# dmiruke/find_motion

Measured on NVIDIA B200. Metric: 1080p frames/sec (whole box), higher is better.
Workload: dtype u8+f64

## Files before the change

### find_motion_b200/csrc/fm_host.cu

```cuda
#include <ctype.h>
#include <math.h>
#include <stdarg.h>
#include <stdio.h>
#include <stdlib.h>
#include <string.h>

#include <algorithm>
#include <map>
#include <mutex>
#include <utility>
#include <vector>

#include <sched.h>
#include <unistd.h>

#include "fm_common.cuh"

std::atomic<unsigned long long> g_launches{0};
static thread_local char g_err[512] = "";

int fm_ensure_smem(const void *func, size_t bytes, int device) {
    static std::mutex mu;
    static std::map<std::pair<const void *, int>, size_t> done;
    std::lock_guard<std::mutex> lk(mu);
// ... 274 lines not shown
        if ((rc = upload(&c->coef, taps))) return fail(rc);
        if (c->umma && (rc = fm_umma_init(c, taps.data()))) return fail(rc);
        if (!c->fused && !c->umma && (rc = fm_wide_init(c, taps.data()))) return fail(rc);
    }

    const size_t F = (size_t)c->S * c->Tmax;
    const size_t flatw = (size_t)c->ntiles * FM_TILE_WORDS;
#define ALLOC(ptr, bytes)                                                                 \
    do {                                                                                  \
        cudaError_t e_ = cudaMalloc((void **)&(ptr), (bytes));                            \
        if (e_ != cudaSuccess) {                                                          \
            fm_set_error("cudaMalloc(%zu bytes) for %s failed: %s", (size_t)(bytes), #ptr, \
                         cudaGetErrorString(e_));                                         \
            return fail(FM_ENOMEM);                                                       \
        }                                                                                 \
    } while (0)
    const bool keep = (cfg->flags & FM_FLAG_KEEP_PLANES) != 0;
    const bool need_gray = keep || !c->fused;
    const bool need_blur = keep || !c->fused;
    ALLOC(c->gray, need_gray ? F * c->N : 16);
    ALLOC(c->hor, (c->fused || c->umma) ? 16 : 2 * fm_wide_plane_bytes(c));
    ALLOC(c->blur, need_blur ? F * c->N + 64 : 64);
    const size_t bg_doubles = std::max((size_t)c->S * c->ntiles * FM_TILE_PX,
                                       c->fused ? fm_fused_bg_doubles(c)
                                                : (c->umma ? fm_umma_bg_doubles(c) : (c->wide_fused ? fm_wide_bg_doubles(c) : (size_t)0)));
    ALLOC(c->bg, bg_doubles * sizeof(double));
    ALLOC(c->maskbits, (size_t)c->S * c->h * c->wpr * 4);
    ALLOC(c->maskflat, (size_t)c->S * flatw * 4);
    ALLOC(c->tflat, (F * flatw + FM_TILE_WORDS) * 4);
    ALLOC(c->dil, F * c->h * c->wpr * 4);
    ALLOC(c->fill, F * c->h * c->wpr * 4);
    ALLOC(c->rawrange, F * 6 * sizeof(int));
    c->any = c->rawrange + 2 * F;
    ALLOC(c->ncomp, (F * 2 + 4) * sizeof(int));
    c->ncounted = c->ncomp + F;
    ALLOC(c->heavy, F * sizeof(int));
    ALLOC(c->comps, F * c->maxc * sizeof(fm_component));
    ALLOC(c->stats, F * sizeof(fm_frame_stats));
    ALLOC(c->state, (size_t)c->S * sizeof(StreamState));
    ALLOC(c->errflag, sizeof(int));
    ALLOC(c->nvalid, (size_t)c->S * sizeof(int));
    c->nvalid_host = (int *)malloc((size_t)c->S * sizeof(int));
    if (!c->nvalid_host) { fm_set_error("out of host memory"); return fail(FM_ENOMEM); }
    for (int s = 0; s < c->S; s++) c->nvalid_host[s] = c->Tmax;
    FM_TRY(cudaMemcpy(c->nvalid, c->nvalid_host, (size_t)c->S * sizeof(int), cudaMemcpyHostToDevice));
    FM_TRY(cudaMemset(c->maskbits, 0, (size_t)c->S * c->h * c->wpr * 4));
    FM_TRY(cudaMemset(c->maskflat, 0, (size_t)c->S * flatw * 4));
    FM_TRY(cudaMemset(c->tflat, 0, (F * flatw + FM_TILE_WORDS) * 4));
    FM_TRY(cudaMemset(c->bg, 0, bg_doubles * sizeof(double)));
    FM_TRY(cudaMemset(c->state, 0, (size_t)c->S * sizeof(StreamState)));
    FM_TRY(cudaMemset(c->errflag, 0, sizeof(int)));
    FM_TRY(cudaMemset(c->heavy, 0, F * sizeof(int)));
    int cap = c->w / 4 + 3;
    size_t per_frame = (size_t)c->h * cap * 28 + (size_t)c->h * 4 + 4;
    size_t budget = (size_t)8 << 30;
    int nb = (int)std::min<size_t>(F, std::max<size_t>(1, budget / per_frame));
    if ((rc = fm_ccl_alloc(&c->ccl, nb, c->h, cap))) return fail(rc);
    if ((rc = fm_ccl_configure(c))) return fail(rc);
    if ((cfg->flags & FM_FLAG_DEVICE_CLIPS) && (rc = fm_clips_alloc(c))) return fail(rc);
    FM_TRY(cudaStreamCreateWithFlags(&c->own_stream, cudaStreamNonBlocking));
    FM_TRY(cudaStreamCreateWithFlags(&c->copy_stream, cudaStreamNonBlocking));
    for (int i = 0; i < 2; i++) {
        FM_TRY(cudaEventCreateWithFlags(&c->ev_copied[i], cudaEventDisableTiming));
        FM_TRY(cudaEventCreateWithFlags(&c->ev_done[i], cudaEventDisableTiming));
    }
#undef FM_TRY
#undef ALLOC
// ... 30 lines not shown
    if (err) {
        FM_CUDA(cudaMemset(c->errflag, 0, sizeof(int)));
        fm_set_error("contour stage: run capacity exceeded (results of the affected frames are not valid)");
        return FM_ERANGE;
    }
    return FM_OK;
}

extern "C" int fm_ctx_set_masks(fm_ctx *c, int stream, int n_polys, const int32_t *poly_offsets,
                                const int32_t *xy) {
    if (!c || n_polys < 0 || (n_polys > 0 && (!poly_offsets || !xy))) { fm_set_error("bad mask arguments"); return FM_EINVAL; }
    if (stream >= c->S) { fm_set_error("stream %d out of range", stream); return FM_EINVAL; }
    FM_CUDA(cudaSetDevice(c->cfg.device));
    FM_CUDA(cudaDeviceSynchronize());
    int npts = n_polys ? poly_offsets[n_polys] : 0;
    std::vector<int> pts((size_t)npts * 2);
    const double scale = c->info.scale;
    for (int i = 0; i < npts * 2; i++) pts[i] = (int)((double)xy[i] * scale);
    int s0 = stream < 0 ? 0 : stream, s1 = stream < 0 ? c->S : stream + 1;
    for (int s = s0; s < s1; s++) {
        int rc = fm_launch_masks(c, s, n_polys, poly_offsets, pts.data(), npts, 0);
        if (rc) return rc;
    }
    FM_CUDA(cudaDeviceSynchronize());
    return FM_OK;
}

static int timing_drain(fm_ctx *c) {
    for (int i = 0; i < c->ev_pending; i++) {
        cudaEvent_t *ev = c->evs + 4 * i;
        FM_CUDA(cudaEventSynchronize(ev[3]));
        for (int g = 0; g < 3; g++) {
            float ms = 0;
            FM_CUDA(cudaEventElapsedTime(&ms, ev[g], ev[g + 1]));
            c->t_ms[g] += ms;
        }
        c->t_calls++;
    }
    c->ev_pending = 0;
    return FM_OK;
}

static int process(fm_ctx *c, const uint8_t *frames, size_t stream_stride, size_t frame_stride, int n_frames,
                   const int32_t *n_valid, void *cuda_stream, fm_frame_stats *stats_dev, uint8_t *out, size_t out_stride) {
    if (!c || !frames) { fm_set_error("null argument"); return FM_EINVAL; }
    if (n_frames < 1 || n_frames > c->Tmax) {
        fm_set_error("n_frames %d outside [1, max_frames=%d]", n_frames, c->Tmax);
        return FM_EINVAL;
    }
    FM_CUDA(cudaSetDevice(c->cfg.device));
    cudaStream_t st = (cudaStream_t)cuda_stream;
    int rc;
    {
        bool changed = false;
        for (int s = 0; s < c->S; s++) {
            int v = n_valid ? n_valid[s] : n_frames;
            if (v < 0 || v > n_frames) { fm_set_error("n_valid[%d] = %d outside [0, n_frames=%d]", s, v, n_frames); return FM_EINVAL; }
            if (v != c->nvalid_host[s]) { c->nvalid_host[s] = v; changed = true; }
        }
        if (changed) FM_CUDA(cudaMemcpyAsync(c->nvalid, c->nvalid_host, (size_t)c->S * sizeof(int), cudaMemcpyHostToDevice, st));
    }
    {
        const size_t Fmax = (size_t)c->S * c->Tmax;
        FM_CUDA(cudaMemsetAsync(c->rawrange, 0xFF, Fmax * 6 * sizeof(int), st));
        FM_CUDA(cudaMemsetAsync(c->ncomp, 0, (Fmax * 2 + 4) * sizeof(int), st));
    }
    cudaEvent_t *ev = nullptr;
    if (c->timing) {
        if (c->ev_pending == FM_TIMING_RING && (rc = timing_drain(c))) return rc;
        ev = c->evs + 4 * c->ev_pending++;
        FM_CUDA(cudaEventRecord(ev[0], st));
    }
    if (c->fused) {
        if ((rc = fm_launch_fused(c, frames, stream_stride, frame_stride, n_frames, st))) return rc;
        if (ev) { FM_CUDA(cudaEventRecord(ev[1], st)); FM_CUDA(cudaEventRecord(ev[2], st)); }
    } else {
        if ((rc = fm_launch_frontend(c, frames, stream_stride, frame_stride, n_frames, st))) return rc;
        if (ev) FM_CUDA(cudaEventRecord(ev[1], st));
        if (!c->wide_fused && !c->umma && (rc = fm_launch_temporal(c, n_frames, st))) return rc;
        if (ev) FM_CUDA(cudaEventRecord(ev[2], st));
    }
    if ((rc = fm_launch_morph_ccl(c, n_frames, st, stats_dev))) return rc;
    if (ev) FM_CUDA(cudaEventRecord(ev[3], st));
    if ((c->cfg.flags & FM_FLAG_DEVICE_CLIPS) &&
        (rc = fm_launch_clips(c, frames, stream_stride, frame_stride, n_frames, out, out_stride, st)))
        return rc;
    c->last_T = n_frames;
    c->planes_valid = true;
    return FM_OK;
}

extern "C" int fm_process_ragged(fm_ctx *c, const uint8_t *frames, size_t stream_stride, size_t frame_stride,
                                 int n_frames, const int32_t *n_valid, void *cuda_stream, fm_frame_stats *stats_dev) {
    return process(c, frames, stream_stride, frame_stride, n_frames, n_valid, cuda_stream, stats_dev, nullptr, 0);
}

extern "C" int fm_process_clip(fm_ctx *c, const uint8_t *frames, size_t stream_stride, size_t frame_stride,
                               int n_frames, const int32_t *n_valid, void *cuda_stream, fm_frame_stats *stats_dev,
                               uint8_t *out_dev, size_t out_stream_stride, int out_capacity) {
    if (!c || !frames || !out_dev) { fm_set_error("null argument"); return FM_EINVAL; }
    if (!(c->cfg.flags & FM_FLAG_DEVICE_CLIPS)) {
        fm_set_error("fm_process_clip needs a context created with FM_FLAG_DEVICE_CLIPS");
        return FM_EINVAL;
    }
    if ((long long)out_capacity < (long long)c->info.cache_frames + n_frames) {
        fm_set_error("out_capacity %d < cache_frames %d + n_frames %d (the most frames one call can write)", out_capacity,
                     c->info.cache_frames, n_frames);
        return FM_EINVAL;
// ... 341 lines not shown
```

### find_motion_b200/csrc/k_morph_ccl.cu

```cuda
#include "fm_common.cuh"

#define WARPS_PER_BLOCK 8

__device__ __forceinline__ uint32_t ld_word(const uint32_t *row, int j, int wpr) {
    return ((unsigned)j < (unsigned)wpr) ? __ldg(row + j) : 0u;
}

__device__ __forceinline__ uint32_t flat_row_word(const uint32_t *flat, int y, int j, int w, int h, int wpr) {
    if ((unsigned)y >= (unsigned)h || (unsigned)j >= (unsigned)wpr) return 0u;
    long long b0 = (long long)y * w + 32 * j;
    int wi = (int)(b0 >> 5), sh = (int)(b0 & 31);
    uint32_t lo = __ldg(flat + wi);
    uint32_t v = lo;
    if (sh) {
        uint32_t hi = __ldg(flat + wi + 1);
        v = __funnelshift_r(lo, hi, sh);
    }
    int rem = w - 32 * j;
    if (rem < 32) v &= (1u << rem) - 1u;
    return v;
}

template <bool ALIGNED>
__device__ __forceinline__ uint32_t dilate_vor(const uint32_t *__restrict__ flat, int y, int j, int w, int h, int wpr) {
    uint32_t v = 0;
    if (j >= wpr) return 0u;
#pragma unroll
    for (int dy = -2; dy <= 2; dy++) {
        const int yy = y + dy;
        if (ALIGNED) {
            if ((unsigned)yy < (unsigned)h) v |= __ldcg(flat + (size_t)yy * wpr + j);
        } else {
            v |= flat_row_word(flat, yy, j, w, h, wpr);
        }
    }
    return v;
}

template <bool ALIGNED>
__device__ __forceinline__ uint32_t dilate_row(const uint32_t *__restrict__ flat, uint32_t *__restrict__ out, int y, int w,
                                               int h, int wpr, int lane, int &jmin, int &jmax) {
    uint32_t anyw = 0, vprev = 0, vc = dilate_vor<ALIGNED>(flat, y, lane, w, h, wpr);
    for (int j0 = 0; j0 < wpr; j0 += 32) {
        const int j = j0 + lane;
        const uint32_t vnext = dilate_vor<ALIGNED>(flat, y, j + 32, w, h, wpr);
        uint32_t vm = __shfl_up_sync(0xffffffffu, vc, 1), vp = __shfl_down_sync(0xffffffffu, vc, 1);
        const uint32_t pl = __shfl_sync(0xffffffffu, vprev, 31), nf = __shfl_sync(0xffffffffu, vnext, 0);
        if (lane == 0) vm = pl;
        if (lane == 31) vp = nf;
        if (j < wpr) {
            uint32_t d = vc | (vc << 1) | (vc << 2) | (vc >> 1) | (vc >> 2) | (vm >> 31) | (vm >> 30) | (vp << 31) | (vp << 30);
            const int rem = w - 32 * j;
            if (rem < 32) d &= (1u << rem) - 1u;
            out[j] = d;
            anyw |= d;
            if (d) { jmax = max(jmax, j); jmin = min(jmin, j); }
        }
        vprev = vc;
        vc = vnext;
    }
    return anyw;
}

template <bool ALIGNED, int NCH>
__device__ __noinline__ void dilate_rows(const uint32_t *flat, uint32_t *dplane, int ya, int yb, int w, int h, int wpr, int lane,
                                            int &jmin, int &jmax, int &ymn, int &ymx) {
    auto raw = [&](int y, int c) -> uint32_t {
        const int j = lane + 32 * c;
        if ((unsigned)y >= (unsigned)h || j >= wpr) return 0u;
        return ALIGNED ? __ldcg(flat + (size_t)y * wpr + j) : flat_row_word(flat, y, j, w, h, wpr);
    };
    uint32_t win[NCH][4];
#pragma unroll
    for (int c = 0; c < NCH; c++)
#pragma unroll
        for (int i = 0; i < 4; i++) win[c][i] = raw(ya - 2 + i, c);
    for (int y0 = ya; y0 < yb; y0 += 4) {
        uint32_t nxt[NCH][4];
#pragma unroll
        for (int c = 0; c < NCH; c++)
#pragma unroll
            for (int i = 0; i < 4; i++) nxt[c][i] = raw(y0 + 2 + i, c);
#pragma unroll
        for (int i = 0; i < 4; i++) {
            const int y = y0 + i;
            if (y >= yb) break;
            uint32_t v[NCH];
#pragma unroll
            for (int c = 0; c < NCH; c++) {
                v[c] = win[c][0] | win[c][1] | win[c][2] | win[c][3] | nxt[c][i];
                win[c][0] = win[c][1]; win[c][1] = win[c][2]; win[c][2] = win[c][3]; win[c][3] = nxt[c][i];
            }
            uint32_t anyw = 0;
#pragma unroll
            for (int c = 0; c < NCH; c++) {
                uint32_t vm = __shfl_up_sync(0xffffffffu, v[c], 1), vp = __shfl_down_sync(0xffffffffu, v[c], 1);
                const uint32_t pl = c > 0 ? __shfl_sync(0xffffffffu, v[c > 0 ? c - 1 : 0], 31) : 0u;
                const uint32_t nf = c + 1 < NCH ? __shfl_sync(0xffffffffu, v[c + 1 < NCH ? c + 1 : c], 0) : 0u;
                if (lane == 0) vm = pl;
                if (lane == 31) vp = nf;
                const int j = lane + 32 * c;
                if (j < wpr) {
                    uint32_t d = v[c] | (v[c] << 1) | (v[c] << 2) | (v[c] >> 1) | (v[c] >> 2) | (vm >> 31) | (vm >> 30) | (vp << 31) | (vp << 30);
                    const int rem = w - 32 * j;
                    if (rem < 32) d &= (1u << rem) - 1u;
                    dplane[(size_t)y * wpr + j] = d;
                    anyw |= d;
                    if (d) { jmax = max(jmax, j); jmin = min(jmin, j); }
                }
            }
            if (__any_sync(0xffffffffu, anyw != 0)) { ymx = max(ymx, y); ymn = min(ymn, y); }
        }
    }
}

template <bool ALIGNED>
__global__ void __launch_bounds__(32 * WARPS_PER_BLOCK) k_dilate(const uint32_t *__restrict__ tflat,
                                                                 uint32_t *__restrict__ dil, int *__restrict__ rowrange,
                                                                 const int *__restrict__ rawrange, int F, int w, int h,
                                                                 int wpr, int flatwords, int T, int t0, int Th) {
    int warp = blockIdx.x * WARPS_PER_BLOCK + (threadIdx.x >> 5);
    int lane = threadIdx.x & 31;
    if (warp >= F * h) return;
    int lf = warp / h, y = warp - lf * h;
    int f = (lf / Th) * T + t0 + lf % Th;
    if (rawrange) {
        int rmax = rawrange[2 * f], rmin = h - 1 - rawrange[2 * f + 1];
        if (rmax < 0 || y < rmin - 3 || y > rmax + 3) return;
    }
    const uint32_t *flat = tflat + (size_t)f * flatwords;
    uint32_t *out = dil + ((size_t)f * h + y) * wpr;
    int jmax = -1, jmin = wpr;
    const uint32_t anyw = dilate_row<ALIGNED>(flat, out, y, w, h, wpr, lane, jmin, jmax);
    if (__any_sync(0xffffffffu, anyw != 0)) {
        jmax = __reduce_max_sync(0xffffffffu, jmax);
        jmin = __reduce_min_sync(0xffffffffu, jmin);
        if (lane == 0) {
            atomicMax(rowrange + 4 * f, y);
            atomicMax(rowrange + 4 * f + 1, h - 1 - y);
            atomicMax(rowrange + 4 * f + 2, jmax);
            atomicMax(rowrange + 4 * f + 3, wpr - 1 - jmin);
        }
    }
}

struct CclArgs {
    const uint32_t *plane;
    uint32_t *fill;
    const int *rowrange;
    const uint32_t *raw;
    const int *rawrange;
    int *rangeout;
    uint32_t *planeout;
    int flatwords, aligned;
    int cache_words;
    int f0, nf;
    int T, t0, Th;
    int w, h, wpr, cap;
    size_t slots;
    uint16_t *xs, *xe;
    int *rowcnt, *parent, *area2, *bbox;
    int *errflag;
    int *ncomp, *ncounted;
    fm_component *comps;
    int maxc, min_area, max_area;
};

template <bool INVERT>
__device__ __forceinline__ uint32_t plane_word(const uint32_t *row, int j, int w, int wpr) {
    if ((unsigned)j >= (unsigned)wpr) return 0u;
    uint32_t v = __ldcg(row + j);
    if (INVERT) {
        v = ~v;
        int rem = w - 32 * j;
        if (rem < 32) v &= (1u << rem) - 1u;
    }
    return v;
}

template <bool INVERT>
__device__ __forceinline__ void runs_row(const CclArgs &a, const uint32_t *plane, int lf, int f, int y, int lane) {
    const uint32_t *row = plane + ((size_t)f * a.h + y) * a.wpr;
    size_t base = (size_t)lf * a.slots + (size_t)y * a.cap;
    int *parent = a.parent + (size_t)lf * (a.slots + 1);
    int nstart = 0, nend = 0;
    for (int j0 = 0; j0 < a.wpr; j0 += 32) {
        int j = j0 + lane;
        uint32_t B = plane_word<INVERT>(row, j, a.w, a.wpr);
        uint32_t Bp = plane_word<INVERT>(row, j - 1, a.w, a.wpr);
        uint32_t Bn = plane_word<INVERT>(row, j + 1, a.w, a.wpr);
        uint32_t S = B & ~((B << 1) | (Bp >> 31));
        uint32_t E = B & ~((B >> 1) | (Bn << 31));
        if (!__any_sync(0xffffffffu, (S | E) != 0)) continue;
        int cs = __popc(S), ce = __popc(E);
        int ps = cs, pe = ce;
#pragma unroll
        for (int o = 1; o < 32; o <<= 1) {
            int vs = __shfl_up_sync(0xffffffffu, ps, o);
            int ve = __shfl_up_sync(0xffffffffu, pe, o);
// ... 154 lines not shown
        if (slot < a.maxc) {
            fm_component c;
            c.area_x2 = area2;
            int x0 = __ldcg(bb), y0 = __ldcg(bb + 1), x1 = __ldcg(bb + 2), y1 = __ldcg(bb + 3);
            c.x = x0; c.y = y0; c.w = x1 - x0 + 1; c.h = y1 - y0 + 1;
            a.comps[(size_t)f * a.maxc + slot] = c;
        }
    }
}

#define CCL_THREADS 1024
__device__ __forceinline__ void ccl_frame_global(const CclArgs &a, int lf, int f, int ylo, int yhi) {
    const int lane = threadIdx.x & 31, warp = threadIdx.x >> 5, nw = CCL_THREADS / 32;
    if (threadIdx.x == 0) a.parent[(size_t)lf * (a.slots + 1)] = 0;
    for (int y = ylo + warp; y <= yhi; y += nw) runs_row<true>(a, a.plane, lf, f, y, lane);
    __syncthreads();
    for (int y = ylo + warp; y <= yhi; y += nw) union_row<false, true>(a, lf, y, ylo, lane);
    __syncthreads();
    for (int y = ylo + warp; y <= yhi; y += nw) fill_row(a, lf, f, y, lane);
    __syncthreads();
    for (int y = ylo + warp; y <= yhi; y += nw) runs_row<false>(a, a.fill, lf, f, y, lane);
    __syncthreads();
    for (int y = ylo + warp; y <= yhi; y += nw) union_row<true, false>(a, lf, y, ylo, lane);
    __syncthreads();
    for (int y = ylo + warp; y <= yhi; y += nw) stats_row(a, lf, f, y, lane);
    __syncthreads();
    for (int y = ylo + warp; y <= yhi; y += nw) collect_row(a, lf, f, y, lane);
}

struct DecideArgs {
    StreamState *state;
    fm_frame_stats *stats, *stats_out;
    const int *nvalid;
    int *done;
    int S, T, total, cache_frames, min_movement_frames;
};

__device__ __forceinline__ void decide_stream(const DecideArgs &d, const int *ncomp, const int *ncounted, int s) {
    StreamState st = d.state[s];
    const int T = d.T;
    const int Ts = min(T, d.nvalid[s]);
    for (int t = Ts; t < T; t++) {
        fm_frame_stats z = {0, 0, 0, 0, 0, 0, 0, 0};
        d.stats[s * T + t] = z;
        if (d.stats_out) d.stats_out[s * T + t] = z;
    }
    if (Ts <= 0) return;
    for (int tc = 0; tc < Ts; tc += 16) {
        int nco[16], ncd[16];
#pragma unroll
        for (int i = 0; i < 16; i++) {
            const bool in = tc + i < Ts;
            nco[i] = in ? __ldcg(ncomp + s * T + tc + i) : 0;
            ncd[i] = in ? __ldcg(ncounted + s * T + tc + i) : 0;
        }
#pragma unroll
        for (int i = 0; i < 16; i++) {
            if (tc + i >= Ts) break;
            const int f = s * T + tc + i;
            fm_frame_stats r;
            r.n_contours = nco[i];
            r.n_counted = ncd[i];
            if (st.decay > 0) st.decay -= 1;
            bool movement = r.n_counted > 0;
            st.counter = movement ? st.counter + r.n_counted : 0;
            r.wrote = 0;
            r.n_flush = 0;
            if (st.counter >= d.min_movement_frames || st.decay > 0) {
                if (movement) {
                    st.decay = d.cache_frames;
                    r.n_flush = st.cache_len;
                    st.cache_len = 0;
                }
                r.wrote = 1;
            } else {
                st.cache_len = min(st.cache_len + 1, d.cache_frames);
            }
            r.movement = movement ? 1 : 0;
            r.movement_counter = st.counter;
            r.movement_decay = st.decay;
            r.cache_len = st.cache_len;
            d.stats[f] = r;
            if (d.stats_out) d.stats_out[f] = r;
        }
    }
    st.has_bg = 1;
    d.state[s] = st;
}

__global__ void k_decide(DecideArgs d, const int *__restrict__ ncomp, const int *__restrict__ ncounted) {
    int s = blockIdx.x * blockDim.x + threadIdx.x;
    if (s < d.S) decide_stream(d, ncomp, ncounted, s);
}

__global__ void __launch_bounds__(CCL_THREADS, 1) k_ccl_frame(CclArgs a, const int *__restrict__ heavy) {
    const int lf = blockIdx.x, lg = a.f0 + lf, f = (lg / a.Th) * a.T + a.t0 + lg % a.Th;
    if (heavy && !heavy[f]) return;
    int ylo = 0, yhi = a.h - 1;
    bool work = true;
    if (a.rowrange) {
        int ymax = a.rowrange[4 * f], ymin = a.h - 1 - a.rowrange[4 * f + 1];
        if (ymax < 0) work = false;
        ylo = max(ymin - 1, 0);
        yhi = min(ymax + 1, a.h - 1);
    }
    if (work) ccl_frame_global(a, lf, f, ylo, yhi);
}

#define CCL2_THREADS 1024
#define CCL2_WARPS (CCL2_THREADS / 32)
#define CCL2_CAP 4096

struct RunTable {
    int2 *row;
    int *parent;
    uint16_t *xs, *xe;
    uint16_t *rowof;
};

__device__ __forceinline__ int suf_find(int *parent, int x) {
    int p = parent[x];
    while (p != x) {
        int gp = parent[p];
        if (gp != p) atomicMin(parent + x, gp);
        x = p;
        p = gp;
    }
    return x;
}

// ... 99 lines not shown
    while (lo < hi) {
        const int mid = (lo + hi) >> 1;
        if ((int)t.xe[prv.x + mid] < xs - d) lo = mid + 1; else hi = mid;
    }
    for (int q = lo; q < prv.y && (int)t.xs[prv.x + q] <= xe + d; q++) {
        if (!linked) {
            if (FIRST) t.parent[id] = id0 + prv.x + q;
            linked = true;
        } else if (!FIRST) {
            suf_union(t.parent, id, id0 + prv.x + q);
            did = true;
        }
    }
    return did;
}

__device__ __forceinline__ void flatten_forest(int *parent, int n) {
    __syncthreads();
    while (true) {
        bool ch = false;
        for (int i = threadIdx.x; i < n; i += CCL2_THREADS) {
            const int p = parent[i];
            int q = parent[p];
            if (q != p) {
                q = parent[parent[q]];
                parent[i] = q;
                ch = true;
            }
        }
        if (!__syncthreads_or(ch)) break;
    }
}

__device__ __forceinline__ bool ccl_frame_lanes(const CclArgs &a, unsigned char *csm, int f, int lf,
                                                int ylo, int yhi, int jlo, int wprw) {
    const int ww = min(a.w - 32 * jlo, 32 * wprw);
    const int nrows = yhi - ylo + 1;
    RunTable bg, fg;
    bg.row = reinterpret_cast<int2 *>(csm);
    fg.row = bg.row + a.h;
    bg.parent = reinterpret_cast<int *>(fg.row + a.h);
    fg.parent = bg.parent + CCL2_CAP + 2;
    bg.xs = reinterpret_cast<uint16_t *>(fg.parent + CCL2_CAP + 2);
    bg.xe = bg.xs + CCL2_CAP;
    fg.xs = bg.xe + CCL2_CAP;
    fg.xe = fg.xs + CCL2_CAP;
    bg.rowof = fg.xe + CCL2_CAP;
    fg.rowof = bg.rowof + CCL2_CAP;
    __shared__ int cur_bg, cur_fg, overflow, wsum[CCL2_WARPS];
    if (threadIdx.x == 0) { cur_bg = 0; cur_fg = 0; overflow = 0; bg.parent[0] = 0; }
    __syncthreads();
    uint32_t *cache = reinterpret_cast<uint32_t *>(fg.rowof + CCL2_CAP);
    const int cpitch = wprw | 1;
    const bool cached = (size_t)nrows * cpitch <= (size_t)a.cache_words;
    const uint32_t *dil;
    uint32_t *fil;
    size_t pitch;
    if (cached) {
        const uint32_t *src = a.plane + ((size_t)f * a.h + ylo) * a.wpr + jlo;
        const int lane = threadIdx.x & 31, warp = threadIdx.x >> 5;
        for (int yr = warp; yr < nrows; yr += CCL2_WARPS)
            for (int j = lane; j < wprw; j += 32) cache[yr * cpitch + j] = __ldcg(src + (size_t)yr * a.wpr + j);
        dil = cache; fil = cache; pitch = cpitch;
        __syncthreads();
    } else {
        dil = a.plane + ((size_t)f * a.h + ylo) * a.wpr + jlo;
        fil = a.fill + ((size_t)f * a.h + ylo) * a.wpr + jlo;
        pitch = a.wpr;
    }

    for (int r0 = 0; r0 < nrows; r0 += CCL2_THREADS) {
        const int yr = r0 + threadIdx.x;
        const bool act = yr < nrows;
        if (!lane_extract<true>(dil + (size_t)(act ? yr : 0) * pitch, act, yr, 1, bg, &cur_bg, wsum, ww, wprw)) overflow = 1;
    }
    __syncthreads();
    if (overflow) return false;
    const int nbg = cur_bg;
    for (int i = threadIdx.x; i < nbg; i += CCL2_THREADS) run_union<false, true, true>(bg, 1, i, ylo, ww, a.h);
    flatten_forest(bg.parent, nbg + 1);
    {
        bool did = false;
        for (int i = threadIdx.x; i < nbg; i += CCL2_THREADS) did |= run_union<false, true, false>(bg, 1, i, ylo, ww, a.h);
        if (__syncthreads_or(did)) flatten_forest(bg.parent, nbg + 1);
    }
    if (!cached) {
        for (int yr = threadIdx.x; yr < nrows; yr += CCL2_THREADS)
            for (int j = 0; j < wprw; j++) fil[(size_t)yr * pitch + j] = dil[(size_t)yr * pitch + j];
        __syncthreads();
    }
    for (int i = threadIdx.x; i < nbg; i += CCL2_THREADS) {
        if (bg.parent[1 + i] == 0) continue;
        const int xs = bg.xs[i], xe = bg.xe[i];
        uint32_t *frow = fil + (size_t)bg.rowof[i] * pitch;
        for (int j = xs >> 5; j <= (xe >> 5); j++) {
            const int lo = max(xs - 32 * j, 0), hi = min(xe - 32 * j, 31);
            atomicOr(frow + j, (hi == 31 ? 0xffffffffu : ((1u << (hi + 1)) - 1u)) & ~((1u << lo) - 1u));
        }
    }
    __syncthreads();
    for (int r0 = 0; r0 < nrows; r0 += CCL2_THREADS) {
        const int yr = r0 + threadIdx.x;
        const bool act = yr < nrows;
        if (!lane_extract<false>(fil + (size_t)(act ? yr : 0) * pitch, act, yr, 0, fg, &cur_fg, wsum, ww, wprw)) overflow = 1;
    }
    __syncthreads();
    if (overflow) return false;
    const int total = cur_fg;
    int *area2 = a.area2 + (size_t)lf * a.slots, *bbox = a.bbox + (size_t)lf * a.slots * 4;
    for (int i = threadIdx.x; i < total; i += CCL2_THREADS) {
        area2[i] = 0;
        reinterpret_cast<int4 *>(bbox)[i] = make_int4(0x7fffffff, 0x7fffffff, -1, -1);
    }
    for (int i = threadIdx.x; i < total; i += CCL2_THREADS) run_union<true, false, true>(fg, 0, i, ylo, ww, a.h);
    flatten_forest(fg.parent, total);
    {
        bool did = false;
        for (int i = threadIdx.x; i < total; i += CCL2_THREADS) did |= run_union<true, false, false>(fg, 0, i, ylo, ww, a.h);
        if (__syncthreads_or(did)) flatten_forest(fg.parent, total);
    }
    for (int i = threadIdx.x; i < total; i += CCL2_THREADS) {
        const int yr = fg.rowof[i], y = ylo + yr;
        const bool has_up = yr > 0;
        const uint32_t *lrow = fil + (size_t)yr * pitch, *urow = lrow - pitch;
        const int xs = fg.xs[i], xe = fg.xe[i];
        const int root = fg.parent[i];
        int q = 0;
        if (has_up) {
            const int x0 = max(xs - 1, 0), x1 = xe;
            uint32_t L = win_word<false>(lrow, x0 >> 5, ww, wprw), U = win_word<false>(urow, x0 >> 5, ww, wprw);
            for (int j = x0 >> 5; j <= (x1 >> 5); j++) {
                const uint32_t Ln = win_word<false>(lrow, j + 1, ww, wprw), Un = win_word<false>(urow, j + 1, ww, wprw);
                const uint32_t l1 = (L >> 1) | (Ln << 31), u1 = (U >> 1) | (Un << 31);
                const uint32_t q4 = L & l1 & U & u1, q3 = (L & l1 & (U ^ u1)) | (U & u1 & (L ^ l1));
                const int lo = max(x0 - 32 * j, 0), hi = min(x1 - 32 * j, 31);
                const uint32_t m = (hi == 31 ? 0xffffffffu : ((1u << (hi + 1)) - 1u)) & ~((1u << lo) - 1u);
                q += 2 * __popc(q4 & m) + __popc(q3 & m);
                L = Ln; U = Un;
            }
        }
        if (q) atomicAdd(area2 + root, q);
        int *bb = bbox + (size_t)root * 4;
        atomicMin(bb + 0, xs);
        atomicMin(bb + 1, y);
        atomicMax(bb + 2, xe);
        atomicMax(bb + 3, y);
    }
    __syncthreads();
    for (int i = threadIdx.x; i < total; i += CCL2_THREADS) {
        if (fg.parent[i] != i) continue;
        const int ar = __ldcg(area2 + i);
        const int4 bb = __ldcg(reinterpret_cast<const int4 *>(bbox) + i);
        const int slot = atomicAdd(a.ncomp + f, 1);
        const bool skipped = (2LL * a.max_area < ar) && (ar < 2LL * a.min_area);
        if (!skipped) atomicAdd(a.ncounted + f, 1);
        if (slot < a.maxc) {
            fm_component c;
            c.area_x2 = ar; c.x = bb.x + 32 * jlo; c.y = bb.y; c.w = bb.z - bb.x + 1; c.h = bb.w - bb.y + 1;
            a.comps[(size_t)f * a.maxc + slot] = c;
        }
    }
    return true;
}

__device__ __forceinline__ bool ccl_window(const CclArgs &a, int f, int &ylo, int &yhi, int &jlo, int &jhi) {
    ylo = 0; yhi = a.h - 1; jlo = 0; jhi = a.wpr - 1;
    if (a.raw) {
        const int rmax = a.rawrange[2 * f], rmin = a.h - 1 - a.rawrange[2 * f + 1];
        if (rmax < 0) return false;
        __shared__ int rng[4];
        if (threadIdx.x < 4) rng[threadIdx.x] = -1;
        __syncthreads();
        const int lane = threadIdx.x & 31, warp = threadIdx.x >> 5;
        const uint32_t *flat = a.raw + (size_t)f * a.flatwords;
        uint32_t *dplane = a.planeout + (size_t)f * a.h * a.wpr;
        int jmax = -1, jmin = a.wpr, ymx = -1, ymn = a.h;
        {
            const int y0 = max(rmin - 3, 0), y1 = min(rmax + 3, a.h - 1) + 1;
            const int B = (y1 - y0 + CCL2_WARPS - 1) / CCL2_WARPS;
            const int ya = y0 + warp * B, yb = min(ya + B, y1);
            if (ya < yb) {
#define FM_DIL(AL, N) dilate_rows<AL, N>(flat, dplane, ya, yb, a.w, a.h, a.wpr, lane, jmin, jmax, ymn, ymx)
                if (a.aligned) { if (a.wpr <= 32) FM_DIL(true, 1); else if (a.wpr <= 64) FM_DIL(true, 2); else FM_DIL(true, 4); }
                else { if (a.wpr <= 32) FM_DIL(false, 1); else if (a.wpr <= 64) FM_DIL(false, 2); else FM_DIL(false, 4); }
#undef FM_DIL
            }
        }
        jmax = __reduce_max_sync(0xffffffffu, jmax);
        jmin = __reduce_min_sync(0xffffffffu, jmin);
        if (lane == 0 && ymx >= 0) {
            atomicMax(&rng[0], ymx);
            atomicMax(&rng[1], a.h - 1 - ymn);
            atomicMax(&rng[2], jmax);
            atomicMax(&rng[3], a.wpr - 1 - jmin);
        }
        __syncthreads();
        if (threadIdx.x < 4) a.rangeout[4 * f + threadIdx.x] = rng[threadIdx.x];
        if (rng[0] < 0) return false;
        ylo = max(a.h - 1 - rng[1] - 1, 0);
        yhi = min(rng[0] + 1, a.h - 1);
        jhi = rng[2];
        jlo = a.wpr - 1 - rng[3];
    } else if (a.rowrange) {
        int ymax = a.rowrange[4 * f], ymin = a.h - 1 - a.rowrange[4 * f + 1];
        if (ymax < 0) return false;
        ylo = max(ymin - 1, 0);
        yhi = min(ymax + 1, a.h - 1);
        jhi = a.rowrange[4 * f + 2];
        jlo = a.wpr - 1 - a.rowrange[4 * f + 3];
    }
    return true;
}

__global__ void __launch_bounds__(CCL2_THREADS, 1) k_ccl_frame_smem(CclArgs a, int *__restrict__ heavy) {
    extern __shared__ __align__(16) unsigned char csm[];
    const int lf = blockIdx.x, lg = a.f0 + lf, f = (lg / a.Th) * a.T + a.t0 + lg % a.Th;
    int ylo, yhi, jlo, jhi;
    bool is_heavy = false;
    if (ccl_window(a, f, ylo, yhi, jlo, jhi)) is_heavy = !ccl_frame_lanes(a, csm, f, lf, ylo, yhi, jlo, jhi - jlo + 1);
    if (threadIdx.x == 0) heavy[f] = is_heavy;
}

__global__ void k_bits_to_u8(const uint32_t *__restrict__ plane, uint8_t *__restrict__ dst, int w, int h, int wpr,
                             uint8_t on, const int *__restrict__ rowrange) {
    int x = blockIdx.x * blockDim.x + threadIdx.x, y = blockIdx.y;
    if (x >= w) return;
    bool live = true;
    if (rowrange) live = rowrange[0] >= 0 && y <= rowrange[0] && y >= h - 1 - rowrange[1];
    dst[(size_t)y * w + x] = (live && ((plane[(size_t)y * wpr + (x >> 5)] >> (x & 31)) & 1u)) ? on : 0;
}

__global__ void k_u8_to_bits(const uint8_t *__restrict__ src, uint32_t *__restrict__ plane, int w, int h, int wpr) {
    int j = blockIdx.x * blockDim.x + threadIdx.x, y = blockIdx.y;
    if (j >= wpr) return;
    uint32_t v = 0;
    for (int b = 0; b < 32; b++) {
        int x = 32 * j + b;
        if (x < w && src[(size_t)y * w + x]) v |= 1u << b;
    }
    plane[(size_t)y * wpr + j] = v;
}

int fm_launch_thresh_export(fm_ctx *c, int stream, int t, uint8_t *dst_dev, cudaStream_t st) {
    const uint32_t *pl = c->dil + ((size_t)stream * c->last_T + t) * c->h * c->wpr;
    dim3 grid((c->w + 127) / 128, c->h);
    k_bits_to_u8<<<grid, 128, 0, st>>>(pl, dst_dev, c->w, c->h, c->wpr, 255, c->any + 4 * ((size_t)stream * c->last_T + t));
    FM_LAUNCH_CHECK();
    return FM_OK;
}

int fm_launch_mask_export(fm_ctx *c, int stream, uint8_t *dst_dev, cudaStream_t st) {
    const uint32_t *pl = c->maskbits + (size_t)stream * c->h * c->wpr;
    dim3 grid((c->w + 127) / 128, c->h);
// ... 10 lines not shown
    FM_CUDA(cudaMalloc(&s->xs, n * sizeof(uint16_t)));
    FM_CUDA(cudaMalloc(&s->xe, n * sizeof(uint16_t)));
    FM_CUDA(cudaMalloc(&s->rowcnt, (size_t)frames * h * sizeof(int)));
    FM_CUDA(cudaMalloc(&s->parent, (size_t)frames * (s->slots + 1) * sizeof(int)));
    FM_CUDA(cudaMalloc(&s->area2, n * sizeof(int)));
    FM_CUDA(cudaMalloc(&s->bbox, n * 4 * sizeof(int)));
    return FM_OK;
}

void fm_ccl_free(CclScratch *s) {
    cudaFree(s->xs); cudaFree(s->xe); cudaFree(s->rowcnt); cudaFree(s->parent); cudaFree(s->area2);
    cudaFree(s->bbox);
    s->xs = s->xe = nullptr; s->rowcnt = s->parent = s->area2 = s->bbox = nullptr;
}

static bool ccl_smem_plan(int h, int wpr, size_t *smem, int *cache_words) {
    const size_t tables = (size_t)2 * h * sizeof(int2) + (size_t)2 * (CCL2_CAP + 2) * sizeof(int) +
                          (size_t)6 * CCL2_CAP * sizeof(uint16_t);
    const size_t budget = 200 * 1024;
    if (wpr > 128 || tables + 4096 > budget) return false;
    const size_t room = budget - tables;
    *smem = tables + (room < 128 * 1024 ? room : 128 * 1024);
    *cache_words = (int)((*smem - tables) / 4);
    return true;
}

int fm_ccl_configure(fm_ctx *c) {
    size_t smem = 0;
    int cw = 0;
    if (!ccl_smem_plan(c->h, c->wpr, &smem, &cw)) return FM_OK;
    return fm_ensure_smem((const void *)k_ccl_frame_smem, smem, c->cfg.device);
}

static int ccl_run(const CclScratch &sc, const uint32_t *plane, uint32_t *fill, int *rowrange, int F, int w,
                   int h, int wpr, int *ncomp, int *ncounted, fm_component *comps, int maxc, int min_area,
                   int max_area, int *errflag, int *heavy, int T, int t0, int Th, cudaStream_t st,
                   const uint32_t *raw = nullptr, const int *rawrange = nullptr, int flatwords = 0) {
    for (int f0 = 0; f0 < F; f0 += sc.frames) {
        int nf = F - f0 < sc.frames ? F - f0 : sc.frames;
        CclArgs a;
        a.plane = plane; a.fill = fill; a.rowrange = rowrange;
        a.raw = raw; a.rawrange = rawrange; a.rangeout = rowrange; a.planeout = const_cast<uint32_t *>(plane);
        a.flatwords = flatwords; a.aligned = (w % 32) == 0;
        a.T = T; a.t0 = t0; a.Th = Th;
        a.f0 = f0; a.nf = nf; a.w = w; a.h = h; a.wpr = wpr; a.cap = sc.cap; a.slots = sc.slots;
        a.xs = sc.xs; a.xe = sc.xe; a.rowcnt = sc.rowcnt; a.parent = sc.parent; a.area2 = sc.area2;
        a.bbox = sc.bbox; a.errflag = errflag;
        a.ncomp = ncomp; a.ncounted = ncounted; a.comps = comps; a.maxc = maxc;
        a.min_area = min_area; a.max_area = max_area;
        a.cache_words = 0;
        size_t smem = 0;
        if (heavy && ccl_smem_plan(h, wpr, &smem, &a.cache_words)) {
            int dev = 0;
            FM_CUDA(cudaGetDevice(&dev));
            int rc = fm_ensure_smem((const void *)k_ccl_frame_smem, smem, dev);
            if (rc) return rc;
            k_ccl_frame_smem<<<nf, CCL2_THREADS, smem, st>>>(a, heavy);
            FM_LAUNCH_CHECK();
            if ((size_t)h * (w / 2 + 2) > CCL2_CAP) k_ccl_frame<<<nf, CCL_THREADS, 0, st>>>(a, heavy);
        } else {
            a.raw = nullptr;
            k_ccl_frame<<<nf, CCL_THREADS, 0, st>>>(a, nullptr);
        }
        FM_LAUNCH_CHECK();
    }
    return FM_OK;
}

int fm_launch_morph_ccl(fm_ctx *c, int T, cudaStream_t st, fm_frame_stats *stats_out) {
    const int F = c->S * T;
    size_t smem_plan = 0;
    int cw_plan = 0, rc;
    const bool smem_ok = ccl_smem_plan(c->h, c->wpr, &smem_plan, &cw_plan);
    if (smem_ok && F >= 32) {
        rc = ccl_run(c->ccl, c->dil, c->fill, c->any, F, c->w, c->h, c->wpr, c->ncomp, c->ncounted, c->comps, c->maxc,
                     c->info.min_area, c->info.max_area, c->errflag, c->heavy, T, 0, T, st, c->tflat, c->rawrange,
                     c->ntiles * FM_TILE_WORDS);
    } else {
        int blocks = (F * c->h + WARPS_PER_BLOCK - 1) / WARPS_PER_BLOCK;
        if (c->w % 32 == 0)
            k_dilate<true><<<blocks, 32 * WARPS_PER_BLOCK, 0, st>>>(c->tflat, c->dil, c->any, c->rawrange, F, c->w, c->h,
                                                                   c->wpr, c->ntiles * FM_TILE_WORDS, T, 0, T);
        else
            k_dilate<false><<<blocks, 32 * WARPS_PER_BLOCK, 0, st>>>(c->tflat, c->dil, c->any, c->rawrange, F, c->w, c->h,
                                                                    c->wpr, c->ntiles * FM_TILE_WORDS, T, 0, T);
        FM_LAUNCH_CHECK();
        rc = ccl_run(c->ccl, c->dil, c->fill, c->any, F, c->w, c->h, c->wpr, c->ncomp, c->ncounted, c->comps, c->maxc,
                     c->info.min_area, c->info.max_area, c->errflag, smem_ok ? c->heavy : nullptr, T, 0, T, st);
    }
    if (rc) return rc;
    DecideArgs d;
    d.state = c->state; d.stats = c->stats; d.stats_out = stats_out; d.nvalid = c->nvalid; d.done = nullptr;
    d.S = c->S; d.T = T; d.total = F; d.cache_frames = c->info.cache_frames; d.min_movement_frames = c->info.min_movement_frames;
    k_decide<<<(c->S + 127) / 128, 128, 0, st>>>(d, c->ncomp, c->ncounted);
    FM_LAUNCH_CHECK();
    return FM_OK;
}

namespace {
struct PlaneScratch {
    CclScratch sc{};
    uint8_t *d8 = nullptr;
    uint32_t *pl = nullptr, *fill = nullptr;
    int *cnt = nullptr;
    fm_component *comps = nullptr;
    ~PlaneScratch() {
        cudaFree(d8); cudaFree(pl); cudaFree(fill); cudaFree(cnt); cudaFree(comps);
        fm_ccl_free(&sc);
    }
};
}

int fm_ccl_plane(int device, const uint8_t *plane_host, int w, int h, int max_n, fm_component *out, int *n) {
    FM_CUDA(cudaSetDevice(device));
    int wpr = (w + 31) / 32;
    PlaneScratch q;
    int rc = fm_ccl_alloc(&q.sc, 1, h, w / 2 + 2);
    if (rc) return rc;
    int maxc = max_n > 0 ? max_n : 1;
    FM_CUDA(cudaMalloc(&q.d8, (size_t)w * h));
    FM_CUDA(cudaMalloc(&q.pl, (size_t)wpr * h * 4));
    FM_CUDA(cudaMalloc(&q.fill, (size_t)wpr * h * 4));
    FM_CUDA(cudaMalloc(&q.cnt, 4 * sizeof(int)));
    FM_CUDA(cudaMalloc(&q.comps, (size_t)maxc * sizeof(fm_component)));
    FM_CUDA(cudaMemcpy(q.d8, plane_host, (size_t)w * h, cudaMemcpyHostToDevice));
    FM_CUDA(cudaMemset(q.cnt, 0, 4 * sizeof(int)));
    dim3 grid((wpr + 63) / 64, h);
// ... 17 lines not shown
```

Baseline: 334,600.

## Add PDL launches, cache dilated rows in smem, and accumulate CCL stats in shared memory

CCL and decide kernels now launch with programmatic dependent launch (griddepcontrol wait/launch) so launch latency overlaps the preceding kernel. The per-frame memset of ncomp/ncounted is removed; kernels now write the counts directly, using shared-memory counters in place of global atomics. Dilated rows are written into the shared-memory cache during windowing so the CCL pass can skip reloading them from global memory, and per-component area/bbox accumulation uses shared-memory int4 slots when they fit. An env-gated clock64 profiling buffer is also added, and the timing bookkeeping for the fused path is adjusted.

```diff
diff --git a/find_motion_b200/csrc/fm_host.cu b/find_motion_b200/csrc/fm_host.cu
--- a/find_motion_b200/csrc/fm_host.cu
+++ b/find_motion_b200/csrc/fm_host.cu
@@ -330,7 +330,7 @@
     ALLOC(c->fill, F * c->h * c->wpr * 4);
     ALLOC(c->rawrange, F * 6 * sizeof(int));
     c->any = c->rawrange + 2 * F;
-    ALLOC(c->ncomp, (F * 2 + 4) * sizeof(int));
+    ALLOC(c->ncomp, F * 2 * sizeof(int));
     c->ncounted = c->ncomp + F;
     ALLOC(c->heavy, F * sizeof(int));
     ALLOC(c->comps, F * c->maxc * sizeof(fm_component));
@@ -427,7 +427,8 @@
         FM_CUDA(cudaEventSynchronize(ev[3]));
         for (int g = 0; g < 3; g++) {
             float ms = 0;
-            FM_CUDA(cudaEventElapsedTime(&ms, ev[g], ev[g + 1]));
+            if (c->fused && g == 1) continue;
+            FM_CUDA(cudaEventElapsedTime(&ms, ev[g == 2 && c->fused ? 1 : g], ev[g + 1]));
             c->t_ms[g] += ms;
         }
         c->t_calls++;
@@ -458,7 +459,6 @@
     {
         const size_t Fmax = (size_t)c->S * c->Tmax;
         FM_CUDA(cudaMemsetAsync(c->rawrange, 0xFF, Fmax * 6 * sizeof(int), st));
-        FM_CUDA(cudaMemsetAsync(c->ncomp, 0, (Fmax * 2 + 4) * sizeof(int), st));
     }
     cudaEvent_t *ev = nullptr;
     if (c->timing) {
@@ -468,7 +468,7 @@
     }
     if (c->fused) {
         if ((rc = fm_launch_fused(c, frames, stream_stride, frame_stride, n_frames, st))) return rc;
-        if (ev) { FM_CUDA(cudaEventRecord(ev[1], st)); FM_CUDA(cudaEventRecord(ev[2], st)); }
+        if (ev) FM_CUDA(cudaEventRecord(ev[1], st));
     } else {
         if ((rc = fm_launch_frontend(c, frames, stream_stride, frame_stride, n_frames, st))) return rc;
         if (ev) FM_CUDA(cudaEventRecord(ev[1], st));
diff --git a/find_motion_b200/csrc/k_morph_ccl.cu b/find_motion_b200/csrc/k_morph_ccl.cu
--- a/find_motion_b200/csrc/k_morph_ccl.cu
+++ b/find_motion_b200/csrc/k_morph_ccl.cu
@@ -1,6 +1,12 @@
+#include <cstdlib>
+#include <cstring>
+
 #include "fm_common.cuh"
 
 #define WARPS_PER_BLOCK 8
+
+__device__ __forceinline__ void grid_dep_wait() { asm volatile("griddepcontrol.wait;" ::: "memory"); }
+__device__ __forceinline__ void grid_dep_launch() { asm volatile("griddepcontrol.launch_dependents;" ::: "memory"); }
 
 __device__ __forceinline__ uint32_t ld_word(const uint32_t *row, int j, int wpr) {
     return ((unsigned)j < (unsigned)wpr) ? __ldg(row + j) : 0u;
@@ -63,8 +69,8 @@
 }
 
 template <bool ALIGNED, int NCH>
-__device__ __noinline__ void dilate_rows(const uint32_t *flat, uint32_t *dplane, int ya, int yb, int w, int h, int wpr, int lane,
-                                            int &jmin, int &jmax, int &ymn, int &ymx) {
+__device__ __noinline__ void dilate_rows(const uint32_t *flat, uint32_t *dplane, uint32_t *srow, int sy0, int spitch, int ya, int yb, int w,
+                                            int h, int wpr, int lane, int &jmin, int &jmax, int &ymn, int &ymx) {
     auto raw = [&](int y, int c) -> uint32_t {
         const int j = lane + 32 * c;
         if ((unsigned)y >= (unsigned)h || j >= wpr) return 0u;
@@ -105,6 +111,7 @@
                     const int rem = w - 32 * j;
                     if (rem < 32) d &= (1u << rem) - 1u;
                     dplane[(size_t)y * wpr + j] = d;
+                    if (srow) srow[(y - sy0) * spitch + j] = d;
                     anyw |= d;
                     if (d) { jmax = max(jmax, j); jmin = min(jmin, j); }
                 }
@@ -164,7 +171,13 @@
     int *ncomp, *ncounted;
     fm_component *comps;
     int maxc, min_area, max_area;
+    long long *prof;
 };
+
+#define CCL_PROF_SLOTS 16
+__device__ __forceinline__ void ccl_stamp(const CclArgs &a, int f, int k, long long v = -1) {
+    if (a.prof && threadIdx.x == 0) a.prof[(size_t)f * CCL_PROF_SLOTS + k] = v < 0 ? clock64() : v;
+}
 
 template <bool INVERT>
 __device__ __forceinline__ uint32_t plane_word(const uint32_t *row, int j, int w, int wpr) {
@@ -385,7 +398,6 @@
     StreamState *state;
     fm_frame_stats *stats, *stats_out;
     const int *nvalid;
-    int *done;
     int S, T, total, cache_frames, min_movement_frames;
 };
 
@@ -442,13 +454,18 @@
 }
 
 __global__ void k_decide(DecideArgs d, const int *__restrict__ ncomp, const int *__restrict__ ncounted) {
+    grid_dep_wait();
+    grid_dep_launch();
     int s = blockIdx.x * blockDim.x + threadIdx.x;
     if (s < d.S) decide_stream(d, ncomp, ncounted, s);
 }
 
 __global__ void __launch_bounds__(CCL_THREADS, 1) k_ccl_frame(CclArgs a, const int *__restrict__ heavy) {
+    grid_dep_wait();
+    grid_dep_launch();
     const int lf = blockIdx.x, lg = a.f0 + lf, f = (lg / a.Th) * a.T + a.t0 + lg % a.Th;
     if (heavy && !heavy[f]) return;
+    if (!heavy && threadIdx.x == 0) { a.ncomp[f] = 0; a.ncounted[f] = 0; }
     int ylo = 0, yhi = a.h - 1;
     bool work = true;
     if (a.rowrange) {
@@ -614,8 +631,13 @@
     }
 }
 
+__device__ __forceinline__ uint32_t *ccl_cache(unsigned char *csm, int h) {
+    return reinterpret_cast<uint32_t *>(csm + (size_t)2 * h * sizeof(int2) + (size_t)2 * (CCL2_CAP + 2) * sizeof(int) +
+                                        (size_t)6 * CCL2_CAP * sizeof(uint16_t));
+}
+
 __device__ __forceinline__ bool ccl_frame_lanes(const CclArgs &a, unsigned char *csm, int f, int lf,
-                                                int ylo, int yhi, int jlo, int wprw) {
+                                                int ylo, int yhi, int jlo, int wprw, int crow0) {
     const int ww = min(a.w - 32 * jlo, 32 * wprw);
     const int nrows = yhi - ylo + 1;
     RunTable bg, fg;
@@ -629,16 +651,20 @@
     fg.xe = fg.xs + CCL2_CAP;
     bg.rowof = fg.xe + CCL2_CAP;
     fg.rowof = bg.rowof + CCL2_CAP;
-    __shared__ int cur_bg, cur_fg, overflow, wsum[CCL2_WARPS];
-    if (threadIdx.x == 0) { cur_bg = 0; cur_fg = 0; overflow = 0; bg.parent[0] = 0; }
-    __syncthreads();
-    uint32_t *cache = reinterpret_cast<uint32_t *>(fg.rowof + CCL2_CAP);
+    __shared__ int cur_bg, cur_fg, overflow, wsum[CCL2_WARPS], nrec, ncnt;
+    if (threadIdx.x == 0) { cur_bg = 0; cur_fg = 0; overflow = 0; bg.parent[0] = 0; nrec = 0; ncnt = 0; }
+    __syncthreads();
+    uint32_t *cache = ccl_cache(csm, a.h);
     const int cpitch = wprw | 1;
-    const bool cached = (size_t)nrows * cpitch <= (size_t)a.cache_words;
+    const bool cached = crow0 >= 0 || (size_t)nrows * cpitch <= (size_t)a.cache_words;
     const uint32_t *dil;
     uint32_t *fil;
     size_t pitch;
-    if (cached) {
+    if (crow0 >= 0) {
+        fil = cache + (size_t)(ylo - crow0) * (a.wpr | 1) + jlo;
+        dil = fil;
+        pitch = a.wpr | 1;
+    } else if (cached) {
         const uint32_t *src = a.plane + ((size_t)f * a.h + ylo) * a.wpr + jlo;
         const int lane = threadIdx.x & 31, warp = threadIdx.x >> 5;
         for (int yr = warp; yr < nrows; yr += CCL2_WARPS)
@@ -650,6 +676,10 @@
         fil = a.fill + ((size_t)f * a.h + ylo) * a.wpr + jlo;
         pitch = a.wpr;
     }
+    ccl_stamp(a, f, 2);
+    ccl_stamp(a, f, 10, nrows);
+    ccl_stamp(a, f, 13, wprw);
+    ccl_stamp(a, f, 14, crow0 >= 0 ? 2 : cached);
 
     for (int r0 = 0; r0 < nrows; r0 += CCL2_THREADS) {
         const int yr = r0 + threadIdx.x;
@@ -659,6 +689,8 @@
     __syncthreads();
     if (overflow) return false;
     const int nbg = cur_bg;
+    ccl_stamp(a, f, 3);
+    ccl_stamp(a, f, 11, nbg);
     for (int i = threadIdx.x; i < nbg; i += CCL2_THREADS) run_union<false, true, true>(bg, 1, i, ylo, ww, a.h);
     flatten_forest(bg.parent, nbg + 1);
     {
@@ -666,6 +698,7 @@
         for (int i = threadIdx.x; i < nbg; i += CCL2_THREADS) did |= run_union<false, true, false>(bg, 1, i, ylo, ww, a.h);
         if (__syncthreads_or(did)) flatten_forest(bg.parent, nbg + 1);
     }
+    ccl_stamp(a, f, 4);
     if (!cached) {
         for (int yr = threadIdx.x; yr < nrows; yr += CCL2_THREADS)
             for (int j = 0; j < wprw; j++) fil[(size_t)yr * pitch + j] = dil[(size_t)yr * pitch + j];
@@ -681,6 +714,7 @@
         }
     }
     __syncthreads();
+    ccl_stamp(a, f, 5);
     for (int r0 = 0; r0 < nrows; r0 += CCL2_THREADS) {
         const int yr = r0 + threadIdx.x;
         const bool act = yr < nrows;
@@ -689,10 +723,20 @@
     __syncthreads();
     if (overflow) return false;
     const int total = cur_fg;
+    ccl_stamp(a, f, 6);
+    ccl_stamp(a, f, 12, total);
+    const size_t used = crow0 >= 0 ? (size_t)(yhi - crow0 + 1) * (a.wpr | 1) : (cached ? (size_t)nrows * cpitch : 0);
+    int4 *acc = nullptr;
+    if (used + 4 * (size_t)total + 4 <= (size_t)a.cache_words)
+        acc = reinterpret_cast<int4 *>(cache + (((size_t)a.cache_words - 4 * (size_t)total) & ~(size_t)3));
     int *area2 = a.area2 + (size_t)lf * a.slots, *bbox = a.bbox + (size_t)lf * a.slots * 4;
     for (int i = threadIdx.x; i < total; i += CCL2_THREADS) {
-        area2[i] = 0;
-        reinterpret_cast<int4 *>(bbox)[i] = make_int4(0x7fffffff, 0x7fffffff, -1, -1);
+        if (acc) {
+            acc[i] = make_int4(0, 0x7fffffff, -1, -1);
+        } else {
+            area2[i] = 0;
+            reinterpret_cast<int4 *>(bbox)[i] = make_int4(0x7fffffff, 0x7fffffff, -1, -1);
+        }
     }
     for (int i = threadIdx.x; i < total; i += CCL2_THREADS) run_union<true, false, true>(fg, 0, i, ylo, ww, a.h);
     flatten_forest(fg.parent, total);
@@ -701,6 +745,7 @@
         for (int i = threadIdx.x; i < total; i += CCL2_THREADS) did |= run_union<true, false, false>(fg, 0, i, ylo, ww, a.h);
         if (__syncthreads_or(did)) flatten_forest(fg.parent, total);
     }
+    ccl_stamp(a, f, 7);
     for (int i = threadIdx.x; i < total; i += CCL2_THREADS) {
         const int yr = fg.rowof[i], y = ylo + yr;
         const bool has_up = yr > 0;
@@ -721,35 +766,59 @@
                 L = Ln; U = Un;
             }
         }
-        if (q) atomicAdd(area2 + root, q);
-        int *bb = bbox + (size_t)root * 4;
-        atomicMin(bb + 0, xs);
-        atomicMin(bb + 1, y);
-        atomicMax(bb + 2, xe);
-        atomicMax(bb + 3, y);
-    }
-    __syncthreads();
+        if (acc) {
+            if (q) atomicAdd(&acc[root].x, q);
+            atomicMin(&acc[root].y, xs);
+            atomicMax(&acc[root].z, xe);
+            atomicMax(&acc[root].w, y);
+        } else {
+            if (q) atomicAdd(area2 + root, q);
+            int *bb = bbox + (size_t)root * 4;
+            atomicMin(bb + 0, xs);
+            atomicMin(bb + 1, y);
+            atomicMax(bb + 2, xe);
+            atomicMax(bb + 3, y);
+        }
+    }
+    __syncthreads();
+    ccl_stamp(a, f, 8);
     for (int i = threadIdx.x; i < total; i += CCL2_THREADS) {
         if (fg.parent[i] != i) continue;
-        const int ar = __ldcg(area2 + i);
-        const int4 bb = __ldcg(reinterpret_cast<const int4 *>(bbox) + i);
-        const int slot = atomicAdd(a.ncomp + f, 1);
+        int ar;
+        int4 bb;
+        if (acc) {
+            const int4 r = acc[i];
+            ar = r.x;
+            bb = make_int4(r.y, ylo + fg.rowof[i], r.z, r.w);
+        } else {
+            ar = __ldcg(area2 + i);
+            bb = __ldcg(reinterpret_cast<const int4 *>(bbox) + i);
+        }
+        const int slot = atomicAdd(&nrec, 1);
         const bool skipped = (2LL * a.max_area < ar) && (ar < 2LL * a.min_area);
-        if (!skipped) atomicAdd(a.ncounted + f, 1);
+        if (!skipped) atomicAdd(&ncnt, 1);
         if (slot < a.maxc) {
             fm_component c;
             c.area_x2 = ar; c.x = bb.x + 32 * jlo; c.y = bb.y; c.w = bb.z - bb.x + 1; c.h = bb.w - bb.y + 1;
             a.comps[(size_t)f * a.maxc + slot] = c;
         }
     }
+    __syncthreads();
+    if (threadIdx.x == 0) { a.ncomp[f] = nrec; a.ncounted[f] = ncnt; }
+    ccl_stamp(a, f, 9);
     return true;
 }
 
-__device__ __forceinline__ bool ccl_window(const CclArgs &a, int f, int &ylo, int &yhi, int &jlo, int &jhi) {
+__device__ __forceinline__ bool ccl_window(const CclArgs &a, uint32_t *cache, int f, int &ylo, int &yhi, int &jlo, int &jhi,
+                                           int &crow0) {
     ylo = 0; yhi = a.h - 1; jlo = 0; jhi = a.wpr - 1;
+    crow0 = -1;
     if (a.raw) {
         const int rmax = a.rawrange[2 * f], rmin = a.h - 1 - a.rawrange[2 * f + 1];
-        if (rmax < 0) return false;
+        if (rmax < 0) {
+            if (threadIdx.x < 4) a.rangeout[4 * f + threadIdx.x] = -1;
+            return false;
+        }
         __shared__ int rng[4];
         if (threadIdx.x < 4) rng[threadIdx.x] = -1;
         __syncthreads();
@@ -761,8 +830,11 @@
             const int y0 = max(rmin - 3, 0), y1 = min(rmax + 3, a.h - 1) + 1;
             const int B = (y1 - y0 + CCL2_WARPS - 1) / CCL2_WARPS;
             const int ya = y0 + warp * B, yb = min(ya + B, y1);
+            const int cp = a.wpr | 1;
+            if ((size_t)(y1 - y0) * cp <= (size_t)a.cache_words) crow0 = y0;
+            uint32_t *srow = crow0 >= 0 ? cache : nullptr;
             if (ya < yb) {
-#define FM_DIL(AL, N) dilate_rows<AL, N>(flat, dplane, ya, yb, a.w, a.h, a.wpr, lane, jmin, jmax, ymn, ymx)
+#define FM_DIL(AL, N) dilate_rows<AL, N>(flat, dplane, srow, y0, cp, ya, yb, a.w, a.h, a.wpr, lane, jmin, jmax, ymn, ymx)
                 if (a.aligned) { if (a.wpr <= 32) FM_DIL(true, 1); else if (a.wpr <= 64) FM_DIL(true, 2); else FM_DIL(true, 4); }
                 else { if (a.wpr <= 32) FM_DIL(false, 1); else if (a.wpr <= 64) FM_DIL(false, 2); else FM_DIL(false, 4); }
 #undef FM_DIL
@@ -796,11 +868,21 @@
 
 __global__ void __launch_bounds__(CCL2_THREADS, 1) k_ccl_frame_smem(CclArgs a, int *__restrict__ heavy) {
     extern __shared__ __align__(16) unsigned char csm[];
+    grid_dep_wait();
+    grid_dep_launch();
     const int lf = blockIdx.x, lg = a.f0 + lf, f = (lg / a.Th) * a.T + a.t0 + lg % a.Th;
     int ylo, yhi, jlo, jhi;
     bool is_heavy = false;
-    if (ccl_window(a, f, ylo, yhi, jlo, jhi)) is_heavy = !ccl_frame_lanes(a, csm, f, lf, ylo, yhi, jlo, jhi - jlo + 1);
-    if (threadIdx.x == 0) heavy[f] = is_heavy;
+    ccl_stamp(a, f, 0);
+    int crow0;
+    const bool work = ccl_window(a, ccl_cache(csm, a.h), f, ylo, yhi, jlo, jhi, crow0);
+    ccl_stamp(a, f, 1);
+    if (work) is_heavy = !ccl_frame_lanes(a, csm, f, lf, ylo, yhi, jlo, jhi - jlo + 1, crow0);
+    ccl_stamp(a, f, 15, work ? 1 + is_heavy : 0);
+    if (threadIdx.x == 0) {
+        heavy[f] = is_heavy;
+        if (!work || is_heavy) { a.ncomp[f] = 0; a.ncounted[f] = 0; }
+    }
 }
 
 __global__ void k_bits_to_u8(const uint32_t *__restrict__ plane, uint8_t *__restrict__ dst, int w, int h, int wpr,
@@ -877,10 +959,44 @@
     return fm_ensure_smem((const void *)k_ccl_frame_smem, smem, c->cfg.device);
 }
 
+#define CCL_PROF_FRAMES 8192
+static long long *g_ccl_prof = nullptr;
+static long long *ccl_prof_buffer() {
+    if (!getenv("FM_CCL_PROF")) return nullptr;
+    if (!g_ccl_prof) {
+        const size_t n = (size_t)CCL_PROF_FRAMES * CCL_PROF_SLOTS;
+        if (cudaMallocManaged(&g_ccl_prof, n * sizeof(long long)) != cudaSuccess) g_ccl_prof = nullptr;
+        else memset(g_ccl_prof, 0xFF, n * sizeof(long long));
+    }
+    return g_ccl_prof;
+}
+
+extern "C" long long *fm_ccl_prof_buffer(int *frames, int *slots) {
+    *frames = CCL_PROF_FRAMES;
+    *slots = CCL_PROF_SLOTS;
+    return g_ccl_prof;
+}
+
+template <typename... KArgs, typename... Args>
+static cudaError_t launch_pdl(void (*kernel)(KArgs...), int grid, int block, size_t smem, cudaStream_t st, bool pdl,
+                              Args... args) {
+    cudaLaunchConfig_t cfg = {};
+    cfg.gridDim = dim3(grid);
+    cfg.blockDim = dim3(block);
+    cfg.dynamicSmemBytes = smem;
+    cfg.stream = st;
+    cudaLaunchAttribute at[1];
+    at[0].id = cudaLaunchAttributeProgrammaticStreamSerialization;
+    at[0].val.programmaticStreamSerializationAllowed = 1;
+    cfg.attrs = at;
+    cfg.numAttrs = pdl ? 1 : 0;
+    return cudaLaunchKernelEx(&cfg, kernel, args...);
+}
+
 static int ccl_run(const CclScratch &sc, const uint32_t *plane, uint32_t *fill, int *rowrange, int F, int w,
                    int h, int wpr, int *ncomp, int *ncounted, fm_component *comps, int maxc, int min_area,
                    int max_area, int *errflag, int *heavy, int T, int t0, int Th, cudaStream_t st,
-                   const uint32_t *raw = nullptr, const int *rawrange = nullptr, int flatwords = 0) {
+                   const uint32_t *raw = nullptr, const int *rawrange = nullptr, int flatwords = 0, bool pdl = false) {
     for (int f0 = 0; f0 < F; f0 += sc.frames) {
         int nf = F - f0 < sc.frames ? F - f0 : sc.frames;
         CclArgs a;
@@ -894,15 +1010,17 @@
         a.ncomp = ncomp; a.ncounted = ncounted; a.comps = comps; a.maxc = maxc;
         a.min_area = min_area; a.max_area = max_area;
         a.cache_words = 0;
+        a.prof = ((F - 1) / Th + 1) * T <= CCL_PROF_FRAMES ? ccl_prof_buffer() : nullptr;
         size_t smem = 0;
         if (heavy && ccl_smem_plan(h, wpr, &smem, &a.cache_words)) {
             int dev = 0;
             FM_CUDA(cudaGetDevice(&dev));
             int rc = fm_ensure_smem((const void *)k_ccl_frame_smem, smem, dev);
             if (rc) return rc;
-            k_ccl_frame_smem<<<nf, CCL2_THREADS, smem, st>>>(a, heavy);
+            FM_CUDA(launch_pdl(k_ccl_frame_smem, nf, CCL2_THREADS, smem, st, pdl, a, heavy));
             FM_LAUNCH_CHECK();
-            if ((size_t)h * (w / 2 + 2) > CCL2_CAP) k_ccl_frame<<<nf, CCL_THREADS, 0, st>>>(a, heavy);
+            if ((size_t)h * (w / 2 + 2) > CCL2_CAP)
+                FM_CUDA(launch_pdl(k_ccl_frame, nf, CCL_THREADS, 0, st, true, a, (const int *)heavy));
         } else {
             a.raw = nullptr;
             k_ccl_frame<<<nf, CCL_THREADS, 0, st>>>(a, nullptr);
@@ -920,7 +1038,7 @@
     if (smem_ok && F >= 32) {
         rc = ccl_run(c->ccl, c->dil, c->fill, c->any, F, c->w, c->h, c->wpr, c->ncomp, c->ncounted, c->comps, c->maxc,
                      c->info.min_area, c->info.max_area, c->errflag, c->heavy, T, 0, T, st, c->tflat, c->rawrange,
-                     c->ntiles * FM_TILE_WORDS);
+                     c->ntiles * FM_TILE_WORDS, true);
     } else {
         int blocks = (F * c->h + WARPS_PER_BLOCK - 1) / WARPS_PER_BLOCK;
         if (c->w % 32 == 0)
@@ -935,9 +1053,9 @@
     }
     if (rc) return rc;
     DecideArgs d;
-    d.state = c->state; d.stats = c->stats; d.stats_out = stats_out; d.nvalid = c->nvalid; d.done = nullptr;
+    d.state = c->state; d.stats = c->stats; d.stats_out = stats_out; d.nvalid = c->nvalid;
     d.S = c->S; d.T = T; d.total = F; d.cache_frames = c->info.cache_frames; d.min_movement_frames = c->info.min_movement_frames;
-    k_decide<<<(c->S + 127) / 128, 128, 0, st>>>(d, c->ncomp, c->ncounted);
+    FM_CUDA(launch_pdl(k_decide, (c->S + 127) / 128, 128, 0, st, true, d, (const int *)c->ncomp, (const int *)c->ncounted));
     FM_LAUNCH_CHECK();
     return FM_OK;
 }
```

Result: faster. 346,700, median of 6 (+3.6%).
